# Yuki-11/CSBSR

Hardware: AMD Instinct MI355X
Metric: training imgs/s (448->1792 x4, PSPNet) (higher is better)
Workload: dtype fp16 storage / fp32 accumulate (detector forward: split fp16 hi+lo); 1 GPU; CSBSR KBPN x4 + PSPNet, beta=0.3, joint phase (iter 40000), per-GPU batch 8, LR 448x448 -> HR 1792x1792, fwd+loss+bwd+Adam; batch resident in HBM (H2D outside `value`, timed beside it as with_h2d_inside_step); full-size synthetic crack images degraded on the device; global_batch=8, micro_batch=8, parallelism=dp1

## Files before the change

### csbsr_amd/_lib.py

```python
import ctypes as C
import os
from collections import namedtuple

import torch

_HERE = os.path.dirname(os.path.abspath(__file__))
LIB_PATH = os.environ.get("CSBSR_LIB") or os.path.join(_HERE, "libcsbsr_hip.so")

ACT_NONE, ACT_RELU, ACT_LRELU, ACT_PRELU, ACT_SIGMOID = 0, 1, 2, 3, 4
RES_NONE, RES_ADD, RES_SUB, RES_MUL, RES_FMA = 0, 1, 2, 3, 4
STAT_NONE, STAT_BN, STAT_SAMPLE_SUM = 0, 1, 2

i32, i64, f32, vp = C.c_int32, C.c_int64, C.c_float, C.c_void_p


class Seg(C.Structure):
    _fields_ = [("ptr", vp), ("sn", i64), ("sy", i64), ("sx", i64), ("c", i32), ("creal", i32)]


class ConvDesc(C.Structure):
    _fields_ = [("inp", Seg * 2), ("N", i32), ("H", i32), ("W", i32), ("OH", i32), ("OW", i32),
                ("transposed", i32), ("KH", i32), ("KW", i32), ("stride", i32), ("pad", i32), ("dil", i32),
                ("wt", vp), ("cout", i32), ("coutp", i32),
                ("out16", vp), ("o_sn", i64), ("o_sy", i64), ("o_sx", i64),
# ... 31 lines not shown
    _fields_ = [("npix", i64), ("hw", i64), ("c", i32), ("creal", i32),
                ("x", vp), ("x_ld", i64), ("mean", vp), ("invstd", vp), ("gamma", vp), ("beta", vp),
                ("res", vp), ("res_ld", i64), ("act", i32), ("_pad", i32), ("prelu", vp), ("drop", vp),
                ("y", vp), ("y_ld", i64), ("dy", vp), ("dy_ld", i64), ("red", vp), ("dprelu", vp),
                ("dx", vp), ("dx_ld", i64), ("dres", vp), ("dres_ld", i64), ("dres_accumulate", i32), ("_pad1", i32),
                ("dgamma", vp), ("dbeta", vp), ("x_lo", i64), ("res_lo", i64), ("y_lo", i64)]


SIGNATURES = {
    "csbsr_version": (i32, []),
    "csbsr_last_error": (C.c_char_p, []),
    "csbsr_conv_forward": (i32, [C.POINTER(ConvDesc), vp]),
    "csbsr_conv_wgrad": (i32, [C.POINTER(WgradDesc), vp]),
    "csbsr_conv_hr_eligible": (i32, [C.POINTER(ConvDesc)]),
    "csbsr_conv_hr_forward": (i32, [C.POINTER(ConvDesc), vp]),
    "csbsr_conv_x3_eligible": (i32, [C.POINTER(ConvDesc)]),
    "csbsr_conv_x3_forward": (i32, [C.POINTER(ConvDesc), vp]),
    "csbsr_packed_weight_elems_x3": (i64, [i32, i32]),
    "csbsr_pack_weights_x3": (i32, [vp, vp, i32, i32, i32, i32, i32, i32, i32, vp]),
    "csbsr_conv_x3n_eligible": (i32, [C.POINTER(ConvDesc)]),
    "csbsr_conv_x3n_forward": (i32, [C.POINTER(ConvDesc), vp]),
    "csbsr_packed_weight_elems_x3n": (i64, [i32, i32]),
    "csbsr_pack_weights_x3n": (i32, [vp, vp, i32, i32, i32, i32, i32, i32, i32, i32, i32, C.c_float, vp]),
    "csbsr_conv_x3w_eligible": (i32, [C.POINTER(ConvDesc)]),
    "csbsr_conv_x3w_forward": (i32, [C.POINTER(ConvDesc), vp]),
    "csbsr_packed_weight_elems_x3w": (i64, [i32, i32]),
    "csbsr_pack_weights_x3w": (i32, [vp, vp, i32, i32, i32, i32, i32, i32, i32, vp]),
    "csbsr_packed_weight_elems_x3_strided": (i64, [i32, i32, i32]),
    "csbsr_pack_weights_x3_strided": (i32, [vp, vp, i32, i32, i32, i32, i32, i32, i32, i32, vp]),
    "csbsr_conv_tp_eligible": (i32, [C.POINTER(ConvDesc)]),
    "csbsr_conv_tp_forward": (i32, [C.POINTER(ConvDesc), vp]),
    "csbsr_packed_weight_elems_tp": (i64, [i32, i32]),
    "csbsr_pack_weights_tp": (i32, [vp, vp, i32, i32, i32, i32, i32, i32, i32, i32, i32, i32, vp]),
    "csbsr_packed_weight_elems_hr": (i64, [i32, i32, i32]),
    "csbsr_pack_weights_hr": (i32, [vp, vp, i32, i32, i32, i32, i32, i32, i32, i32, vp]),
    "csbsr_packed_weight_elems": (i64, [i32] * 9),
    "csbsr_pack_weights": (i32, [vp, vp] + [i32] * 12 + [vp]),
    "csbsr_packed_weight_elems_split": (i64, [i32] * 9),
    "csbsr_pack_weights_split": (i32, [vp, vp] + [i32] * 11 + [f32, i32, vp]),
    "csbsr_axpby_split": (i32, [i64, i32, vp, i64, i64, f32, vp, i64, i64, f32, vp, i64, i64, vp]),
    "csbsr_nchw32_to_nhwc16_split": (i32, [vp, vp, i32, i32, i32, i32, i32, i64, i64, vp, vp, vp]),
    "csbsr_maxpool3x3s2_fwd_split": (i32, [vp, i64, i64, vp, i64, i64, i32, i32, i32, i32, vp]),
    "csbsr_maxpool3x3s2_bwd_split": (i32, [vp, i64, i64, vp, i64, i64, vp, vp, i32, i32, i32, i32, vp]),
    "csbsr_adaptive_avgpool_fwd_split": (i32, [vp, i64, i64, vp, i64, i64, i32, i32, i32, i32, i32, i32, vp]),
    "csbsr_sum_act_split": (i32, [i64, i32, i32, vp, vp, vp, vp, i64, i64, i32, vp]),
    "csbsr_weighted_pool_fwd_split": (i32, [vp, i64, i64, vp, vp, i32, i64, i32, vp]),
    "csbsr_bilinear_fwd_split": (i32, [vp, i64, i64, vp, i64, i64, i32, i32, i32, i32, i32, i32, i32, vp, vp]),
    "csbsr_unpack_wgrad": (i32, [vp, vp] + [i32] * 9 + [f32, i32, i32, vp]),
    "csbsr_wgrad_splits": (i32, [i32, i32, i64]),
    "csbsr_wgrad_splits_desc": (i32, [vp]),
    "csbsr_epilogue_backward": (i32, [C.POINTER(EpiBwdDesc), vp]),
    "csbsr_set_reduction_scratch": (i32, [vp, i64]),
    "csbsr_axpby": (i32, [i64, i32, vp, i64, f32, vp, i64, f32, vp, i64, vp]),
    "csbsr_fill_f16": (i32, [vp, i64, i32, i64, f32, vp]),
    "csbsr_sum_act": (i32, [i64, i32, i32, vp, vp, vp, i64, i32, vp]),
    "csbsr_weighted_pool_fwd": (i32, [vp, i64, vp, vp, i32, i64, i32, vp]),
    "csbsr_weighted_pool_bwd": (i32, [vp, i64, vp, vp, vp, i64, vp, i32, i64, i32, vp]),
    "csbsr_nchw32_to_nhwc16": (i32, [vp, vp, i32, i32, i32, i32, i32, i64, vp, vp, vp]),
    "csbsr_nhwc16_to_nchw32": (i32, [vp, i64, vp, i32, i32, i32, i32, f32, f32, vp]),
    "csbsr_plane_reduce": (i32, [vp, vp, i32, i64, vp, vp]),
    "csbsr_channel_mean_sub": (i32, [vp, i64, i64, i64, i32, i32, i32, i32, i32, vp, vp]),
    "csbsr_thin_tp_backward_slabs": (i32, [i32, i32]),
    "csbsr_conv_thin_dact_eligible": (i32, [vp]),
    "csbsr_conv_split_fused_eligible": (i32, [C.POINTER(ConvDesc)]),
    "csbsr_thin_tp_backward": (i32, [vp, i64, i64, i64, vp, i64, i64, i64, vp, i32, i32, i32, i32, vp, i32, i32, i32, vp, i64, i64, i64, vp, vp, vp]),
    "csbsr_conv_pair1x1_slabs": (i32, [i32, i32, i32, vp]),
    "csbsr_conv_pair1x1_backward": (i32, [vp, i64, i64, i64, vp, i64, i64, i64, vp, f32, i32, i32, i32, vp, i64, i64, i64, vp, vp]),
    "csbsr_round_weights": (i32, [vp, vp, vp, i32, i32, i32, i32, i32, vp]),
    "csbsr_dc_bias": (i32, [vp, i32, i32, vp, i64, i32, vp, i64, i32, vp, i32, vp, vp]),
    "csbsr_instnorm_bwd": (i32, [vp, i64, vp, vp, vp, vp, i32, i32, i32, i64, vp, vp]),
    "csbsr_border_class_fill": (i32, [vp, vp, i64, i32, i32, i32, i32, vp]),
    "csbsr_border_class_fill_masked": (i32, [vp, vp, i64, vp, i64, C.c_float, i32, i32, i32, i32, vp]),
    "csbsr_border_class_sums": (i32, [vp, i64, vp, i32, i32, i32, i32, vp]),
    "csbsr_border_class_fill_masked_sums": (i32, [vp, vp, i64, vp, i64, C.c_float, vp, i32, i32, i32, i32, vp]),
    "csbsr_border_class_sums_prelu": (i32, [vp, i64, vp, i64, vp, vp, i32, i32, i32, i32, vp]),
    "csbsr_ring_class_sums": (i32, [vp, i64, vp, i32, i32, i32, i32, vp]),
    "csbsr_bn_finalize": (i32, [vp, i64, i32, i32, f32, f32, vp, vp, vp, vp, vp]),
    "csbsr_bn_apply": (i32, [C.POINTER(BnDesc), vp]),
    "csbsr_bn_backward": (i32, [C.POINTER(BnDesc), vp]),
    "csbsr_maxpool3x3s2_fwd": (i32, [vp, vp, i32, i32, i32, i32, vp]),
    "csbsr_maxpool3x3s2_bwd": (i32, [vp, vp, vp, vp, i32, i32, i32, i32, vp]),
    "csbsr_adaptive_avgpool_fwd": (i32, [vp, i64, vp, i32, i32, i32, i32, i32, i32, vp]),
    "csbsr_adaptive_avgpool_bwd": (i32, [vp, vp, i64, i32, i32, i32, i32, i32, i32, i32, vp]),
    "csbsr_bilinear_fwd": (i32, [vp, i64, vp, i64, i32, i32, i32, i32, i32, i32, i32, vp, vp]),
    "csbsr_bilinear_bwd": (i32, [vp, i64, vp, i64, i32, i32, i32, i32, i32, i32, i32, i32, vp, vp]),
    "csbsr_bilinear32_fwd": (i32, [vp, vp, i32, i32, i32, i32, i32, i32, vp]),
    "csbsr_bilinear32_bwd": (i32, [vp, vp, i32, i32, i32, i32, i32, i32, vp]),
    "csbsr_bicubic_up_add": (i32, [vp, vp, i32, i32, i32, i32, vp]),
    "csbsr_aa_bicubic_up": (i32, [vp, vp, i32, i32, i32, i32, i32, i32, vp]),
    "csbsr_aa_bicubic_down_fwd": (i32, [vp, vp, i32, i32, i32, i32, i32, vp]),
    "csbsr_aa_bicubic_down_bwd": (i32, [vp, vp, i32, i32, i32, i32, i32, i32, vp]),
    "csbsr_area_down_fwd": (i32, [vp, vp, i32, i32, i32, i32, vp]),
    "csbsr_area_down_bwd": (i32, [vp, vp, i32, i32, i32, i32, i32, vp]),
    "csbsr_blur_fwd": (i32, [vp, vp, i32, i32, i32, i32, i32, i32, vp, vp, vp, i64, vp]),
    "csbsr_blur_bwd_input": (i32, [vp, vp, vp, i32, i32, i32, i32, i32, i32, i32, vp]),
    "csbsr_blur_bwd_kernel": (i32, [vp, vp, vp, i32, i32, i32, i32, i32, i32, vp]),
    "csbsr_sdf": (i32, [vp, vp, vp, i32, i32, i32, vp]),
    "csbsr_crack_weight": (i32, [vp, vp, vp, vp, i32, i32, i32, f32, f32, i32, vp]),
    "csbsr_segloss_reduce": (i32, [vp, vp, vp, i32, i64, vp, f32, f32, vp]),
    "csbsr_segloss_finish": (i32, [vp, vp, vp, i32, i64, vp, f32, f32, f32, f32, f32, f32, vp, vp, vp, i32, vp]),
    "csbsr_l1_fwd_bwd": (i32, [vp, vp, vp, i32, i32, i64, vp, f32, vp, vp, i32, vp]),
    "csbsr_sigmoid_bwd_to_nhwc8": (i32, [vp, vp, vp, i64, f32, vp]),
    "csbsr_gaussian_kernels": (i32, [vp, vp, i32, i32, vp]),
    "csbsr_gather_crop_u8": (i32, [vp, vp, vp, i32, vp, i32, i32, i32, vp, vp]),
    "csbsr_gather_resize_u8": (i32, [vp, vp, vp, i32, vp, i32, i32, i32, i32, vp, vp]),
    "csbsr_stitch_clip_u8": (i32,[vp, i32, i32, i32, i32, i32, i32, i32, vp, vp, vp]),
    "csbsr_stitch_tiles_u8": (i32, [vp, i32, i32, i32, i32, vp, vp, vp, i32, vp, vp, vp]),
    "csbsr_threshold_planes_u8": (i32, [vp, vp, i32, i64, i32, vp, vp]),
    "csbsr_iou_sweep": (i32, [vp, vp, vp, i32, i64, i32, f32, vp, vp, vp, vp, vp]),
    "csbsr_psnr_ssim": (i32, [vp, vp, i32, i32, i32, i32, vp, vp, vp, vp]),
    "csbsr_surface_prepare": (i32, [vp, vp, vp, i32, i32, i32, vp, vp, vp, vp, vp, vp, vp]),
    "csbsr_surface_gather": (i32, [vp, vp, vp, vp, i32, i32, i32, i32, vp, vp, vp, vp, vp, i32, vp, i32, vp, vp]),
    "csbsr_pr_sweep": (i32, [vp, vp, vp, i32, i32, i32, i32, i32, vp, vp, vp]),
    "csbsr_skeleton_max_passes": (i32, []),
    "csbsr_skeleton_init": (i32, [vp, f32, i32, i32, i32, vp, vp]),
    "csbsr_skeleton_passes": (i32, [vp, vp, i32, i32, i32, i32, vp, vp]),
    "csbsr_skeleton_finish": (i32, [vp, i32, i32, i32, vp, vp]),
    "csbsr_centerline_counts": (i32, [vp, vp, f32, vp, vp, i32, i32, i32, vp, vp]),
    "csbsr_ccl_tile": (i32, [C.POINTER(i32), C.POINTER(i32)]),
    "csbsr_ccl_label": (i32, [vp, f32, i32, i32, i32, i32, vp, vp, vp]),
    "csbsr_component_sums": (i32, [vp, vp, i32, i32, i32, vp, vp]),
    "csbsr_component_keep": (i32, [vp, vp, i32, i32, i32, i32, vp, vp, vp]),
    "csbsr_width_max_radius": (i32, []),
    "csbsr_width_tile": (i32, [C.POINTER(i32), C.POINTER(i32)]),
    "csbsr_skeleton_width": (i32, [vp, f32, vp, i32, i32, i32, i32, vp, vp, vp]),
    "csbsr_component_width": (i32, [vp, vp, i32, i32, i32, vp, vp]),
    "csbsr_skeleton_topology": (i32, [vp, i32, i32, i32, vp, vp, vp]),
    "csbsr_component_topology": (i32, [vp, vp, vp, i32, i32, i32, vp, vp]),
    "csbsr_branch_tile": (i32, [C.POINTER(i32), C.POINTER(i32)]),
    "csbsr_branch_label": (i32, [vp, i32, i32, i32, vp, vp, vp]),
    "csbsr_branch_sums": (i32, [vp, vp, vp, vp, i32, i32, i32, vp, vp]),
    "csbsr_prune_max_spur": (i32, []),
    "csbsr_prune_steps": (i32, [C.POINTER(i32), C.POINTER(i32)]),
    "csbsr_prune_tile": (i32, [C.POINTER(i32), C.POINTER(i32)]),
    "csbsr_prune_work_bytes": (i64, [i32, i32, i32]),
    "csbsr_skeleton_prune": (i32, [vp, i32, i32, i32, i32, vp, vp, vp, vp, vp]),
    "csbsr_head1_fwd":(i32, [vp, i64, i64, i32, vp, vp, i32, vp, i64, vp]),
    "csbsr_head1_bwd_input": (i32, [vp, i64, vp, i32, vp, i64, i64, vp]),
    "csbsr_adam_step": (i32, [vp, vp, vp, i32, C.c_double, C.c_double, C.c_float, vp]),
    "csbsr_sgd_step": (i32, [vp, vp, vp, i32, C.c_double, C.c_double, C.c_double, vp]),
    "csbsr_fingerprint": (i32, [vp, vp, vp, i32, vp, vp]),
}

DEBUG_SIGNATURES = {
    "csbsr_debug_set_wgrad_tr": (None, [i32]),
    "csbsr_debug_set_conv_glds": (None, [i32]),
    "csbsr_debug_set_conv_tp": (None, [i32]),
    "csbsr_debug_set_conv_x3": (None, [i32]),
    "csbsr_debug_set_conv_x3w": (None, [i32]),
    "csbsr_debug_set_conv_x3n": (None, [i32]),
    "csbsr_debug_set_wgrad_hr": (None, [i32]),
    "csbsr_debug_last_conv_kernel": (i32, []),
    "csbsr_debug_last_wgrad_kernel": (i32, []),
    "csbsr_debug_cu_trace": (i32, [vp, i32, i32, vp]),
    "csbsr_debug_stream_create_cu_mask": (i32, [C.POINTER(vp), C.POINTER(C.c_uint32), i32]),
    "csbsr_debug_stream_destroy": (i32, [vp]),
    "csbsr_debug_stream_set_cu_budget": (i32, [vp, i32]),
    "csbsr_debug_stream_cu_budget": (i32, [vp]),
}

Hook = namedtuple("Hook", "var default attr parse setter setter_parse", defaults=(None, None, None, None, int))
_not0, _is1 = "0".__ne__, "1".__eq__
ENV_HOOKS = (
    Hook("CSBSR_WGRAD_DBG", setter="csbsr_debug_set_wgrad_tr"),
    Hook("CSBSR_CONV_X3", "1", "use_x3", _not0, "csbsr_debug_set_conv_x3"),
    Hook("CSBSR_CONV_X3W", "0", "use_x3w", lambda v: {"0": 0, "all": 2}.get(v, 1), "csbsr_debug_set_conv_x3w", lambda v: 1 if v == "all" else int(v)),
# ... 52 lines not shown
```

### csbsr_amd/modeling/pspnet.py

```python
import os

import torch

from .. import _lib as L
from ..engine import FM, Conv, _ptr
from .blocks import ConvBN, act_bwd, sft_bwd
from .kbpn import border_tap_mask
from .shapes import RESNET34

DROP_P = {"drop_1": 0.3, "drop_2a": 0.15, "drop_2b": 0.15, "drop_2c": 0.15, "aux_drop": 0.1}
DROP_C = {"drop_1": 1024, "drop_2a": 256, "drop_2b": 64, "drop_2c": 64, "aux_drop": 256}


class _SFTLike:

    def __init__(self, eng, P, pre, cf, cconst):
        def mk(name, act, prelu):
            return Conv(eng, f"{pre}.{name}.layer", P, 3, 1, 1, bias=True, act=act, prelu=f"{pre}.{name}.act.weight" if prelu else False,
                        split=(cf, cconst) if prelu else None)
        self.sc0, self.sc1 = mk("conv_scale.0", L.ACT_PRELU, True), mk("conv_scale.1", L.ACT_SIGMOID, False)
        self.sh0, self.sh1 = mk("conv_shift.0", L.ACT_PRELU, True), mk("conv_shift.1", L.ACT_NONE, False)

    def convs(self):
        return [self.sc0, self.sc1, self.sh0, self.sh1]


class _ResBlock:

    def __init__(self, eng, P, pre, stride, dil, down, layer):
        self.eng, self.layer = eng, layer
        self.c1 = ConvBN(eng, P, pre + ".conv1", pre + ".bn1", 3, stride, dil, dil)
        self.c2 = ConvBN(eng, P, pre + ".conv2", pre + ".bn2", 3, 1, dil, dil)
        self.down = ConvBN(eng, P, pre + ".downsample.0", pre + ".downsample.1", 1, stride, 0, act=L.ACT_NONE) if down else None

    def units(self):
        return [self.c1, self.c2] + ([self.down] if self.down else [])

    def fwd(self, x, training, tape, out=None):
        a1 = self.c1.fwd(x, training, tape)
        pre = self.c2.conv_stats(a1, training)
        res = self.down.fwd(x, training, tape) if self.down else x
        return self.c2.fwd(a1, training, tape, res=res, out=out, pre=pre)

    def bwd(self, tape, dy):
        dres = self.eng.new(dy.N, dy.H, dy.W, dy.c)
        da1 = self.c2.bwd(tape, dy, dres=dres)
        g1 = self.c1.bwd_bn(tape, da1)
        del da1
        dx = self.down.bwd(tape, dres) if self.down else dres
        self.c1.bwd_dx(g1, out=dx, acc=True)
        return dx


class PSPNet:
    drop_keys = tuple(DROP_P)

    def __init__(self, eng, params, prefix="segmentation_model", blur_dim=None):
        self.eng, self.P, self.prefix = eng, params, prefix
        self.blur_dim = blur_dim
        self.blur_skip = []
        e, P, f = eng, params, prefix + ".feats"
        if blur_dim is not None:
            for i in range(2):
                bs = f"{prefix}.blur_skip.{2 * i + 1}"
                self.blur_skip.append((_SFTLike(e, P, f"{prefix}.blur_skip.{2 * i}", 64, blur_dim), ConvBN(e, P, bs + ".layer", bs + ".norm", 3)))
            self.Mtap = border_tap_mask().to(eng.device)
        self.stem = ConvBN(e, P, f + ".conv1", f + ".bn1", 7, 2)
        self.blocks = []
        inpl = 64
        for li, (planes, nblk, stride, dil) in enumerate(RESNET34, 1):
            for b in range(nblk):
                s_, d_ = (stride, 1) if b == 0 else (1, dil)
                self.blocks.append(_ResBlock(e, P, f"{f}.layer{li}.{b}", s_, d_, b == 0 and (stride != 1 or inpl != planes), li))
            inpl = planes
        self.x3_block = [b for b in self.blocks if b.layer == 3][-1]
        self.psp_convs = [Conv(e, f"{prefix}.psp.stages.{i}.1", P, 1, bias=False) for i in range(4)]
        self.bottleneck = Conv(e, prefix + ".psp.bottleneck", P, 1, bias=True, act=L.ACT_RELU)
        self.ups = [ConvBN(e, P, f"{prefix}.{n}.conv.0", f"{prefix}.{n}.conv.1", 3, bias=True, act=L.ACT_PRELU, prelu=P[f"{prefix}.{n}.conv.2.weight"])
                    for n in ("up_1", "up_2", "up_3")]
        self.final = Conv(e, prefix + ".final.0", P, 1, bias=True, act=L.ACT_SIGMOID)
        self.aux0 = ConvBN(e, P, prefix + ".aux.0", prefix + ".aux.1", 3)
        self.aux4 = Conv(e, prefix + ".aux.4", P, 1, bias=True, act=L.ACT_SIGMOID)
        self.saved = None
        self.split = False
        self.split_tail_plain = int(os.environ.get("CSBSR_SPLIT_TAIL_PLAIN", "0"))

    def all_convs(self):
        cs = [u.conv for u in [self.stem] + [u for b in self.blocks for u in b.units()]]
        cs += self.psp_convs + [self.bottleneck] + [u.conv for u in self.ups] + [self.final, self.aux0.conv, self.aux4]
        for sft, cb in self.blur_skip:
            cs += sft.convs() + [cb.conv]
        return cs

    def invalidate(self):
        for c in self.all_convs():
            c.invalidate()

    def make_dropout(self, B, training, enabled=True):
        if not training or not enabled:
            return {k: None for k in DROP_P}
        out = {}
        for k, p in DROP_P.items():
            keep = (torch.rand(B, DROP_C[k], device=self.eng.device) >= p).to(torch.float32) / (1.0 - p)
            out[k] = keep.contiguous()
        return out

    def forward(self, xin, drop, training=True, kvec=None):
        e = self.eng
        B, H, W = xin.N, xin.H, xin.W
        tape = {} if training and torch.is_grad_enabled() else None
        trunk = tape if self.blur_dim is None else None
        a = self.stem.fwd(xin, training, trunk)
        PH, PW = (a.H + 2 - 3) // 2 + 1, (a.W + 2 - 3) // 2 + 1
        x = e.new(B, PH, PW, 64, split=bool(a.lo))
        L.call("csbsr_maxpool3x3s2_fwd_split", _ptr(a.t), a.ld, a.lo, _ptr(x.t), x.ld, x.lo, B, a.H, a.W, 64, e.stream)
        pool = (a, x)
        for blk in self.blocks:
            out = None
            if blk is self.blocks[-1]:
                cat = e.new(B, x.H, x.W, 2560, split=bool(x.lo))
                out = cat.slice(2048, 2560)
            x = blk.fwd(x, training, trunk, out=out)
            if blk is self.x3_block:
                x3 = x
        fH, fW = x.H, x.W
        psp = []
        for i, size in enumerate((1, 2, 3, 6)):
            pooled = e.new(B, size, size, 512, split=bool(x.lo))
            L.call("csbsr_adaptive_avgpool_fwd_split", _ptr(x.t), x.ld, x.lo, _ptr(pooled.t), pooled.ld, pooled.lo, B, fH, fW, 512, size, size,
                   e.stream)
            pc = self.psp_convs[i].fwd(pooled)
            e.bilinear(pc, fH, fW, False, out=cat.slice(512 * i, 512 * (i + 1)))
            psp.append((pooled, pc))
        bott = self.bottleneck.fwd(cat)
        cur, cur_drop = bott, drop["drop_1"]
        ups = []
        for j, (up, name) in enumerate(zip(self.ups, ("drop_2a", "drop_2b", "drop_2c"))):
            if cur.lo and j >= len(self.ups) - self.split_tail_plain:
                cur = FM(cur.t, cur.c, H=cur.H, W=cur.W)
            u = e.bilinear(cur, cur.H * 2, cur.W * 2, False, drop=cur_drop)
            ups.append((cur, cur_drop))
            cur, cur_drop = up.fwd(u, training, trunk, drop=drop[name] if j == 2 else None), drop[name]
        if trunk is not None:
            tape.update(pool=pool, psp=(cat, psp, bott), ups=ups)
        if self.blur_dim is not None:
            cur = self._blur_skip_fwd(cur, kvec, training, tape)
        seg32 = e.f32(B, 1, H, W, zero=False)
        self.final.fwd(cur, out32=seg32)
        aa = self.aux0.fwd(x3, training, trunk, drop=drop["aux_drop"])
        aux_lo = e.f32(B, 1, x3.H, x3.W, zero=False)
        self.aux4.fwd(aa, out32=aux_lo)
        aux32 = e.f32(B, 1, H, W, zero=False)
        L.call("csbsr_bilinear32_fwd", _ptr(aux_lo), _ptr(aux32), B, x3.H, x3.W, H, W, 1, e.stream)
        if tape is not None:
            tape.update(seg32=seg32, p3=cur)
        if trunk is not None:
            tape["aux"] = (aa, aux_lo)
        self.saved = tape
        return seg32, aux32

    def _blur_skip_fwd(self, p, kvec, training, tape):
        e = self.eng
        q, bsv = p, []
        for sft, cb in self.blur_skip:
            t1, f1 = sft.sc0.fwd_folded(q, kvec, self.Mtap)
            sc = sft.sc1.fwd(t1)
            t2, f2 = sft.sh0.fwd_folded(q, kvec, self.Mtap)
            y = sft.sh1.fwd(t2, res=q, res2=sc, res_mode=L.RES_FMA)
            bsv.append((q, (t1, f1, sc, t2, f2, y)))
            q = cb.fwd(y, training, tape)
        out = e.new(p.N, p.H, p.W, p.c, split=bool(p.lo))
        L.call("csbsr_axpby_split", p.npix, p.cp, _ptr(p.t), p.ld, p.lo, 1.0, _ptr(q.t), q.ld, q.lo, 1.0, _ptr(out.t), out.ld, out.lo,
               e.stream)
        if tape is not None:
            tape["blur_skip"] = bsv
        return out

    def _blur_skip_bwd(self, tape, d):
        bsv = tape.pop("blur_skip")
        for i in (1, 0):
            sft, cb = self.blur_skip[i]
            q, saves = bsv.pop()
            dy = cb.bwd(tape, d)
            del d
            dq = self.eng.new(q.N, q.H, q.W, q.c) if i > 0 else None
            sft_bwd(sft.sc0, sft.sc1, sft.sh0, sft.sh1, saves, q, dy, self.Mtap, dx=dq)
            del dy, saves
            d = dq

    def _sigmoid_head_bwd(self, conv, dprob32, prob32, x, frozen=False):
        e = self.eng
        B, _, H, W = prob32.shape
        dpre = e.new(B, H, W, 1)
        L.call("csbsr_sigmoid_bwd_to_nhwc8", _ptr(dprob32), _ptr(prob32), _ptr(dpre.t), B * H * W, 1.0, e.stream)
        if not frozen:
            act_bwd(conv, dpre)
            conv.bwd_weights(dpre, x)
        return conv.bwd_input(dpre)

    def backward(self, dseg32, daux32, need_dxin=True):
        e = self.eng
        tape, self.saved = self.saved, None
        B, _, H, W = dseg32.shape
        if self.blur_dim is not None:
            self._blur_skip_bwd(tape, self._sigmoid_head_bwd(self.final, dseg32, tape.pop("seg32"), tape.pop("p3"), frozen=True))
            return None
        aa, aux_lo = tape.pop("aux")
        daux_lo = e.f32(B, 1, *aux_lo.shape[2:], zero=False)
        L.call("csbsr_bilinear32_bwd", _ptr(daux32), _ptr(daux_lo), B, *aux_lo.shape[2:], H, W, 1, e.stream)
        dx3_aux = self.aux0.bwd(tape, self._sigmoid_head_bwd(self.aux4, daux_lo, aux_lo, aa))
        del aa
        d = self._sigmoid_head_bwd(self.final, dseg32, tape.pop("seg32"), tape.pop("p3"))
        ups = tape.pop("ups")
        for up in reversed(self.ups):
            cur, cur_drop = ups.pop()
            du = up.bwd(tape, d)
            d = e.new(B, cur.H, cur.W, cur.c)
            e.bilinear_bwd(du, d, False, False, drop=cur_drop)
            del du, cur
        cat, psp, bott = tape.pop("psp")
        act_bwd(self.bottleneck, d, bott)
        self.bottleneck.bwd_weights(d, cat)
        dcat = self.bottleneck.bwd_input(d)
        del d, bott
        fH, fW = cat.H, cat.W
        dy = dcat.slice(2048, 2560)
        for i, size in enumerate((1, 2, 3, 6)):
            pooled, pc = psp[i]
            dpc = e.new(B, size, size, 512)
            e.bilinear_bwd(dcat.slice(512 * i, 512 * (i + 1)), dpc, False, False)
            self.psp_convs[i].bwd_weights(dpc, pooled)
            dpool = self.psp_convs[i].bwd_input(dpc)
            L.call("csbsr_adaptive_avgpool_bwd", _ptr(dpool.t), _ptr(dy.t), dy.ld, 1, B, fH, fW, 512, size, size, e.stream)
        del cat, psp
        for blk in reversed(self.blocks):
            if blk is self.x3_block:
                L.call("csbsr_axpby", dy.npix, dy.cp, _ptr(dy.t), dy.ld, 1.0, _ptr(dx3_aux.t), dx3_aux.ld, 1.0, _ptr(dy.t), dy.ld, e.stream)
            dy = blk.bwd(tape, dy)
        a, p = tape.pop("pool")
        da = e.new(B, a.H, a.W, 64)
        assert dy.flat_ok() and dy.ld == dy.cp
        L.call("csbsr_maxpool3x3s2_bwd_split", _ptr(a.t), a.ld, a.lo, _ptr(p.t), p.ld, p.lo, _ptr(dy.t), _ptr(da.t), B, a.H, a.W, 64, e.stream)
        return self.stem.bwd(tape, da, need_dx=need_dxin)
```

### include/csbsr_hip.h

```cpp
#ifndef CSBSR_HIP_H
#define CSBSR_HIP_H
#include <stdint.h>
#ifdef __cplusplus
extern "C" {
#endif

typedef void* csbsr_stream_t;

int csbsr_version(void);
const char* csbsr_last_error(void);

enum { CSBSR_ACT_NONE = 0, CSBSR_ACT_RELU = 1, CSBSR_ACT_LRELU = 2, CSBSR_ACT_PRELU = 3, CSBSR_ACT_SIGMOID = 4 };
enum { CSBSR_RES_NONE = 0, CSBSR_RES_ADD = 1, CSBSR_RES_SUB = 2, CSBSR_RES_MUL = 3, CSBSR_RES_FMA = 4 };
enum { CSBSR_STAT_NONE = 0, CSBSR_STAT_BN = 1 ,
       CSBSR_STAT_SAMPLE_SUM = 2  };

typedef struct {
  const void* ptr;
  int64_t sn, sy, sx;
  int32_t c;
  int32_t creal;
} csbsr_seg_t;

typedef struct {
// ... 148 lines not shown

int csbsr_axpby_split(int64_t npix, int32_t c, const void* x, int64_t x_ld, int64_t x_lo, float a, const void* z, int64_t z_ld,
                      int64_t z_lo, float b, void* y, int64_t y_ld, int64_t y_lo, csbsr_stream_t s);
int csbsr_nchw32_to_nhwc16_split(const float* src, void* dst, int32_t N, int32_t C, int32_t H, int32_t W, int32_t cp,
                                 int64_t dst_ld, int64_t dst_lo, const float* mean, const float* invstd, csbsr_stream_t s);
int csbsr_maxpool3x3s2_fwd_split(const void* x, int64_t x_ld, int64_t x_lo, void* y, int64_t y_ld, int64_t y_lo, int32_t N,
                                 int32_t H, int32_t W, int32_t c, csbsr_stream_t s);
int csbsr_maxpool3x3s2_bwd_split(const void* x, int64_t x_ld, int64_t x_lo, const void* y, int64_t y_ld, int64_t y_lo,
                                 const void* dy, void* dx, int32_t N, int32_t H, int32_t W, int32_t c, csbsr_stream_t s);
int csbsr_adaptive_avgpool_fwd_split(const void* x, int64_t x_ld, int64_t x_lo, void* y, int64_t y_ld, int64_t y_lo, int32_t N,
                                     int32_t H, int32_t W, int32_t c, int32_t OH, int32_t OW, csbsr_stream_t s);
int csbsr_sum_act_split(int64_t npix, int32_t c, int32_t n, const void* const* xs, const int64_t* x_lds, const int64_t* x_los, void* y,
                        int64_t y_ld, int64_t y_lo, int32_t relu, csbsr_stream_t s);
int csbsr_weighted_pool_fwd_split(const void* x, int64_t x_ld, int64_t x_lo, const float* w, float* out, int32_t N, int64_t hw,
                                  int32_t c, csbsr_stream_t s);
int csbsr_bilinear_fwd_split(const void* x, int64_t x_ld, int64_t x_lo, void* y, int64_t y_ld, int64_t y_lo, int32_t N, int32_t H,
                             int32_t W, int32_t c, int32_t OH, int32_t OW, int32_t align_corners, const float* drop,
                             csbsr_stream_t s);

int csbsr_sum_act(int64_t npix, int32_t c, int32_t n, const void* const* xs, const int64_t* x_lds, void* y, int64_t y_ld,
                  int32_t relu, csbsr_stream_t s);
int csbsr_weighted_pool_fwd(const void* x, int64_t x_ld, const float* w, float* out, int32_t N, int64_t hw, int32_t c,
                            csbsr_stream_t s);
int csbsr_weighted_pool_bwd(const void* x, int64_t x_ld, const float* w, const float* dout, void* dx, int64_t dx_ld, float* dw,
                            int32_t N, int64_t hw, int32_t c, csbsr_stream_t s);

int csbsr_nchw32_to_nhwc16(const float* src, void* dst, int32_t N, int32_t C, int32_t H, int32_t W, int32_t cp,
                           int64_t dst_ld, const float* mean, const float* invstd, csbsr_stream_t s);
int csbsr_nhwc16_to_nchw32(const void* src, int64_t src_ld, float* dst, int32_t N, int32_t C, int32_t H, int32_t W,
                           float alpha, float beta, csbsr_stream_t s);
int csbsr_plane_reduce(const float* a, const float* b, int32_t planes, int64_t hw, float* out, csbsr_stream_t s);
int csbsr_channel_mean_sub(const void* x, int64_t sn, int64_t sy, int64_t sx, int32_t N, int32_t H, int32_t W, int32_t cp,
                           int32_t step, float* out, csbsr_stream_t s);
int csbsr_round_weights(const float* w, float* wq, float* S, int32_t D0, int32_t D1, int32_t KH, int32_t KW, int32_t mode, csbsr_stream_t s);
int csbsr_dc_bias(const float* S, int32_t cout, int32_t cin, const float* m0, int64_t m0_ld, int32_t c0, const float* m1, int64_t m1_ld,
                  int32_t c1, const float* bias, int32_t N, float* out, csbsr_stream_t s);
int csbsr_instnorm_bwd(const void* dy, int64_t dy_ld, const float* x, const float* mean, const float* invstd,
                       float* dx, int32_t accumulate, int32_t N, int32_t C, int64_t hw, float* red,
                       csbsr_stream_t s);

int csbsr_border_class_fill(const float* V, void* out, int64_t ld, int32_t N, int32_t H, int32_t W, int32_t c,
                            csbsr_stream_t s);
int csbsr_border_class_fill_masked(const float* V, void* out, int64_t ld, const void* mask, int64_t mask_ld, float mask_slope, int32_t N,
                                   int32_t H, int32_t W, int32_t c, csbsr_stream_t s);
int csbsr_border_class_sums(const void* x, int64_t ld, float* sums, int32_t N, int32_t H, int32_t W, int32_t c,
                            csbsr_stream_t s);
int csbsr_border_class_fill_masked_sums(const float* V, void* out, int64_t ld, const void* mask, int64_t mask_ld, float mask_slope,
                                        float* sums, int32_t N, int32_t H, int32_t W, int32_t c, csbsr_stream_t s);
int csbsr_border_class_sums_prelu(const void* x, int64_t ld, const void* t, int64_t t_ld, float* sums, float* negdot, int32_t N, int32_t H,
                                  int32_t W, int32_t c, csbsr_stream_t s);
int csbsr_ring_class_sums(const void* x, int64_t ld, float* sums, int32_t N, int32_t H, int32_t W, int32_t c,
                          csbsr_stream_t s);

int csbsr_bn_finalize(const float* stat, int64_t count, int32_t c, int32_t cstride, float eps, float momentum,
                      float* mean, float* invstd, float* running_mean, float* running_var, csbsr_stream_t s);
typedef struct {
  int64_t npix, hw;
  int32_t c, creal;
  const void* x; int64_t x_ld;
  const float *mean, *invstd, *gamma, *beta;
  const void* res; int64_t res_ld;
  int32_t act; int32_t _pad;
  const float* prelu;
  const float* drop;
  void* y; int64_t y_ld;
  const void* dy; int64_t dy_ld;
  float* red;
  float* dprelu;
  void* dx; int64_t dx_ld;
  void* dres; int64_t dres_ld; int32_t dres_accumulate; int32_t _pad1;
  float *dgamma, *dbeta;
  int64_t x_lo, res_lo, y_lo;
} csbsr_bn_desc_t;
int csbsr_bn_apply(const csbsr_bn_desc_t* d, csbsr_stream_t s);
int csbsr_bn_backward(const csbsr_bn_desc_t* d, csbsr_stream_t s);

int csbsr_maxpool3x3s2_fwd(const void* x, void* y, int32_t N, int32_t H, int32_t W, int32_t c, csbsr_stream_t s);
int csbsr_maxpool3x3s2_bwd(const void* x, const void* y, const void* dy, void* dx, int32_t N, int32_t H, int32_t W,
                           int32_t c, csbsr_stream_t s);
int csbsr_adaptive_avgpool_fwd(const void* x, int64_t x_ld, void* y, int32_t N, int32_t H, int32_t W, int32_t c,
                               int32_t OH, int32_t OW, csbsr_stream_t s);
int csbsr_adaptive_avgpool_bwd(const void* dy, void* dx, int64_t dx_ld, int32_t accumulate, int32_t N, int32_t H,
                               int32_t W, int32_t c, int32_t OH, int32_t OW, csbsr_stream_t s);
int csbsr_bilinear_fwd(const void* x, int64_t x_ld, void* y, int64_t y_ld, int32_t N, int32_t H, int32_t W,
                       int32_t c, int32_t OH, int32_t OW, int32_t align_corners, const float* drop, csbsr_stream_t s);
int csbsr_bilinear_bwd(const void* dy, int64_t dy_ld, void* dx, int64_t dx_ld, int32_t accumulate, int32_t N,
                       int32_t H, int32_t W, int32_t c, int32_t OH, int32_t OW, int32_t align_corners,
                       const float* drop, csbsr_stream_t s);
int csbsr_bilinear32_fwd(const float* x, float* y, int32_t planes, int32_t H, int32_t W, int32_t OH, int32_t OW,
                         int32_t align_corners, csbsr_stream_t s);
int csbsr_bilinear32_bwd(const float* dy, float* dx, int32_t planes, int32_t H, int32_t W, int32_t OH, int32_t OW,
                         int32_t align_corners, csbsr_stream_t s);
int csbsr_bicubic_up_add(const float* x, float* out, int32_t planes, int32_t H, int32_t W, int32_t scale,
                         csbsr_stream_t s);
int csbsr_aa_bicubic_up(const float* x, float* y, int32_t planes, int32_t H, int32_t W, int32_t scale,
                        int32_t antialias, int32_t clip, csbsr_stream_t s);
int csbsr_aa_bicubic_down_fwd(const float* x, float* y, int32_t planes, int32_t H, int32_t W, int32_t f,
                              int32_t antialias, csbsr_stream_t s);
int csbsr_aa_bicubic_down_bwd(const float* dy, float* dx, int32_t accumulate, int32_t planes, int32_t H, int32_t W,
                              int32_t f, int32_t antialias, csbsr_stream_t s);
int csbsr_area_down_fwd(const float* x, float* y, int32_t planes, int32_t H, int32_t W, int32_t f, csbsr_stream_t s);
int csbsr_area_down_bwd(const float* dy, float* dx, int32_t accumulate, int32_t planes, int32_t H, int32_t W, int32_t f,
                        csbsr_stream_t s);

int csbsr_blur_fwd(const float* x, const float* kvec, int32_t N, int32_t C, int32_t H, int32_t W, int32_t K,
                   int32_t stride, const float* sub, float* y32, void* y16, int64_t y16_ld, csbsr_stream_t s);
int csbsr_blur_bwd_input(const float* dy, const float* kvec, float* dx, int32_t accumulate, int32_t N, int32_t C,
                         int32_t H, int32_t W, int32_t K, int32_t stride, csbsr_stream_t s);
int csbsr_blur_bwd_kernel(const float* dy, const float* x, float* dk, int32_t N, int32_t C, int32_t H, int32_t W,
                          int32_t K, int32_t stride, csbsr_stream_t s);

int csbsr_sdf(const float* mask, float* sdf, float* scratch, int32_t N, int32_t H, int32_t W, csbsr_stream_t s);
int csbsr_crack_weight(const float* mask, float* w_hr, float* w_lr, float* scratch, int32_t N, int32_t H, int32_t W,
                       float amp, float lambda, int32_t scale, csbsr_stream_t s);
int csbsr_segloss_reduce(const float* p, const float* t, const float* sdf, int32_t N, int64_t hw, float* sums,
                         float pw0, float pw1, csbsr_stream_t s);
int csbsr_segloss_finish(const float* p, const float* t, const float* sdf, int32_t N, int64_t hw, const float* sums,
                         float alpha, float pw0, float pw1, float lw0, float lw1, float weight, const float* gscale,
                         float* loss, float* dp, int32_t dp_accumulate, csbsr_stream_t s);
int csbsr_l1_fwd_bwd(const float* a, const float* b, const float* wmap, int32_t N, int32_t C, int64_t hw,
                     float* sums, float gscale, const float* gs_n, float* da, int32_t da_accumulate, csbsr_stream_t s);
int csbsr_sigmoid_bwd_to_nhwc8(const float* dp, const float* p, void* out, int64_t npix, float scale,
                               csbsr_stream_t s);

int csbsr_head1_fwd(const void* x, int64_t ld, int64_t lo, int32_t c, const float* w, const float* bias, int32_t sigmoid, float* out,
                    int64_t npix, csbsr_stream_t s);
int csbsr_head1_bwd_input(const void* dpre, int64_t dpre_ld, const float* w, int32_t c, void* dx, int64_t ld, int64_t npix, csbsr_stream_t s);

int csbsr_gaussian_kernels(const float* params, float* out, int32_t N, int32_t K, csbsr_stream_t s);
int csbsr_gather_crop_u8(const uint8_t* pool, const int64_t* offsets, const int32_t* dims, int32_t channels, const int32_t* sel,
                         int32_t B, int32_t h, int32_t w, float* out, csbsr_stream_t s);
int csbsr_gather_resize_u8(const uint8_t* pool, const int64_t* offsets, const int32_t* dims, int32_t channels, const int32_t* sel,
                           int32_t B, int32_t h, int32_t w, int32_t antialias, float* out, csbsr_stream_t s);
int csbsr_stitch_clip_u8(const float* patches, int32_t B, int32_t C, int32_t nH, int32_t nW, int32_t ph, int32_t pw, int32_t clip,
                         float* out_f32, uint8_t* out_u8, csbsr_stream_t s);
int csbsr_stitch_tiles_u8(const float* patches, int32_t N, int32_t C, int32_t PH, int32_t PW, const int32_t* tiles, const int64_t* offsets,
                          const int32_t* dims, int32_t clip, float* out_f32, uint8_t* out_u8, csbsr_stream_t s);
int csbsr_threshold_planes_u8(const float* pred, const float* thresholds, int32_t N, int64_t hw, int32_t S, uint8_t* out, csbsr_stream_t s);
int csbsr_iou_sweep(const float* pred, const float* mask, const float* thresholds, int32_t N, int64_t hw, int32_t T, float smooth,
                    uint32_t* hist, float* iou, float* inter, float* uni, csbsr_stream_t s);
int csbsr_psnr_ssim(const float* a, const float* b, int32_t N, int32_t C, int32_t H, int32_t W, float* sums, float* psnr, float* ssim,
                    csbsr_stream_t s);

int csbsr_surface_prepare(const float* pred, const float* mask, const float* thresholds, int32_t H, int32_t W, int32_t T, uint8_t* lvl,
                          uint8_t* gt, int32_t* counts, int32_t* rowflag, uint16_t* gcol, int32_t* dgt, csbsr_stream_t s);
int csbsr_surface_gather(const uint8_t* lvl, const uint8_t* gt, const int32_t* dgt, const int32_t* rowflag, int32_t H, int32_t W, int32_t j0,
                         int32_t nj, uint16_t* gcol, const int32_t* tab_off, const int32_t* tab_cap, int32_t* tab_keys, uint32_t* tab_cnt,
                         int32_t max_cap, int32_t* rows, int32_t max_rows, int32_t* meta, csbsr_stream_t s);

int csbsr_pr_sweep(const float* pred, const float* mask, const float* thresholds, int32_t N, int32_t H, int32_t W, int32_t T, int32_t tol2,
                   uint32_t* hist, int32_t* counts, csbsr_stream_t s);

int32_t csbsr_skeleton_max_passes(void);
int csbsr_skeleton_init(const float* planes, float threshold, int32_t N, int32_t H, int32_t W, uint32_t* work, csbsr_stream_t s);
int csbsr_skeleton_passes(const uint32_t* src, uint32_t* dst, int32_t N, int32_t H, int32_t W, int32_t passes, int32_t* deleted,
                          csbsr_stream_t s);
int csbsr_skeleton_finish(const uint32_t* work, int32_t N, int32_t H, int32_t W, uint8_t* out, csbsr_stream_t s);
int csbsr_centerline_counts(const uint8_t* skel_pred, const float* pred, float threshold, const uint8_t* skel_gt, const float* mask, int32_t N,
                            int32_t H, int32_t W, int32_t* counts, csbsr_stream_t s);

int csbsr_ccl_tile(int32_t* th, int32_t* tw);
int csbsr_ccl_label(const float* planes, float threshold, int32_t N, int32_t H, int32_t W, int32_t connectivity, int32_t* work,
                    int32_t* labels, csbsr_stream_t s);
int csbsr_component_sums(const int32_t* labels, const uint8_t* skeleton, int32_t N, int32_t H, int32_t W, int32_t* acc, csbsr_stream_t s);
int csbsr_component_keep(const int32_t* labels, const int32_t* acc, int32_t N, int32_t H, int32_t W, int32_t min_px, uint8_t* keep,
                         int32_t* labels_out, csbsr_stream_t s);
// ... 39 lines not shown
```

Measured before the change: 8.296 imgs/s.

## Fuse PSP pyramid pooling and bilinear backward across all four levels

```diff
diff --git a/csbsr_amd/_lib.py b/csbsr_amd/_lib.py
--- a/csbsr_amd/_lib.py
+++ b/csbsr_amd/_lib.py
@@ -137,6 +137,9 @@
     "csbsr_maxpool3x3s2_bwd": (i32, [vp, vp, vp, vp, i32, i32, i32, i32, vp]),
     "csbsr_adaptive_avgpool_fwd": (i32, [vp, i64, vp, i32, i32, i32, i32, i32, i32, vp]),
     "csbsr_adaptive_avgpool_bwd": (i32, [vp, vp, i64, i32, i32, i32, i32, i32, i32, i32, vp]),
+    "csbsr_psp_pool_fwd": (i32, [vp, i64, i64, vp, vp, vp, i32, i32, i32, i32, vp]),
+    "csbsr_psp_pool_bwd": (i32, [vp, vp, i64, i32, i32, i32, i32, i32, vp]),
+    "csbsr_psp_bilinear_bwd": (i32, [vp, i64, vp, vp, i32, i32, i32, i32, vp]),
     "csbsr_bilinear_fwd": (i32, [vp, i64, vp, i64, i32, i32, i32, i32, i32, i32, i32, vp, vp]),
     "csbsr_bilinear_bwd": (i32, [vp, i64, vp, i64, i32, i32, i32, i32, i32, i32, i32, i32, vp, vp]),
     "csbsr_bilinear32_fwd": (i32, [vp, vp, i32, i32, i32, i32, i32, i32, vp]),
diff --git a/csbsr_amd/csrc/psp_passes.hip b/csbsr_amd/csrc/psp_passes.hip
--- /dev/null
+++ b/csbsr_amd/csrc/psp_passes.hip
@@ -0,0 +1,261 @@
+#include "common.h"
+
+#define ST(s) reinterpret_cast<hipStream_t>(s)
+#define PSP_LEVELS 4
+#define PSP_BINS 50
+#define PSP_BATCH 8
+
+static __host__ __device__ __forceinline__ int prior(int l) { return l == 3 ? 6 : l + 1; }
+static __device__ __forceinline__ int bin_first(int l) { return l == 0 ? 0 : l == 1 ? 1 : l == 2 ? 5 : 14; }
+static __device__ __forceinline__ int level_of_bin(int b) { return b < 1 ? 0 : b < 5 ? 1 : b < 14 ? 2 : 3; }
+static __device__ __forceinline__ int bin_lo(int o, int n, int S) { return (o * n) / S; }
+static __device__ __forceinline__ int bin_hi(int o, int n, int S) { return ((o + 1) * n + S - 1) / S; }
+
+static __device__ __forceinline__ void st_split(half_t* p, long lo, const float (&v)[8]) {
+  h8 a, b;
+#pragma unroll
+  for (int e = 0; e < 8; ++e) { a[e] = (half_t)v[e]; b[e] = (half_t)(v[e] - (float)a[e]); }
+  *reinterpret_cast<h8*>(p) = a;
+  if (lo) *reinterpret_cast<h8*>(p + lo) = b;
+}
+static __device__ __forceinline__ void bil_src(int o, int in, int out, int& i0, int& i1, float& w1) {
+  float src = (o + 0.5f) * ((float)in / (float)out) - 0.5f;
+  if (src < 0.f) src = 0.f;
+  i0 = (int)src; if (i0 > in - 1) i0 = in - 1;
+  i1 = i0 + 1 < in ? i0 + 1 : in - 1;
+  w1 = src - i0;
+}
+
+struct PspMaps { half_t* p[PSP_LEVELS]; long ld[PSP_LEVELS]; long lo[PSP_LEVELS]; };
+struct PspGrads { const half_t* p[PSP_LEVELS]; };
+struct PspSlices { const half_t* p[PSP_LEVELS]; int scan[PSP_LEVELS]; };
+
+static __device__ __forceinline__ void psp_block(int N, int groups, int& n, int& g, int& l, int& o0, int& o1) {
+  int b = blockIdx.x;
+  g = b % groups; b /= groups;
+  n = b % N; b /= N;
+  l = level_of_bin(b);
+  o0 = (b - bin_first(l)) / prior(l); o1 = (b - bin_first(l)) % prior(l);
+}
+static __device__ __forceinline__ float lane_sum(const float (*sred)[8][8], int cl, int e) {
+  float s_ = 0.f;
+  for (int q = 0; q < 32; ++q) s_ += sred[q][cl][e];
+  return s_;
+}
+
+__global__ __launch_bounds__(256) void psp_pool_fwd_kernel(const half_t* x, long x_ld, long x_lo, const PspMaps out, int N, int H, int W, int c8) {
+  __shared__ float sred[32][8][8];
+  int n, g, l, oy, ox;
+  psp_block(N, (c8 + 7) / 8, n, g, l, oy, ox);
+  const int S = prior(l);
+  const int cl = threadIdx.x & 7, pl = threadIdx.x >> 3;
+  const int cc = g * 8 + cl;
+  const int y0 = bin_lo(oy, H, S), y1 = bin_hi(oy, H, S);
+  const int x0 = bin_lo(ox, W, S), x1 = bin_hi(ox, W, S);
+  const int bw = x1 - x0, cnt = (y1 - y0) * bw;
+  const bool block = (long)(H / S) * (W / S) >= 64;
+  const int step = block ? 32 : 1, first = block ? pl : (pl == 0 ? 0 : cnt);
+  float a[8];
+#pragma unroll
+  for (int e = 0; e < 8; ++e) a[e] = 0.f;
+  if (cc < c8) {
+    const half_t* base = x + (long)n * H * W * x_ld + cc * 8;
+    for (int i0 = first; i0 < cnt; i0 += step * PSP_BATCH) {
+      h8 vh[PSP_BATCH], vl[PSP_BATCH];
+#pragma unroll
+      for (int u = 0; u < PSP_BATCH; ++u) {
+        const int i = i0 + u * step;
+        if (i < cnt) {
+          const half_t* p = base + ((long)(y0 + i / bw) * W + (x0 + i % bw)) * x_ld;
+          vh[u] = *reinterpret_cast<const h8*>(p);
+          if (x_lo) vl[u] = *reinterpret_cast<const h8*>(p + x_lo);
+        }
+      }
+#pragma unroll
+      for (int u = 0; u < PSP_BATCH; ++u)
+        if (i0 + u * step < cnt) {
+          float v[8];
+#pragma unroll
+          for (int e = 0; e < 8; ++e) v[e] = (float)vh[u][e];
+          if (x_lo) {
+#pragma unroll
+            for (int e = 0; e < 8; ++e) v[e] += (float)vl[u][e];
+          }
+#pragma unroll
+          for (int e = 0; e < 8; ++e) a[e] += v[e];
+        }
+    }
+  }
+#pragma unroll
+  for (int e = 0; e < 8; ++e) sred[pl][cl][e] = a[e];
+  __syncthreads();
+  if (pl == 0 && cc < c8) {
+    half_t* q = out.p[l] + (((long)n * S + oy) * S + ox) * out.ld[l] + cc * 8;
+    if (block) {
+      float o[8];
+#pragma unroll
+      for (int e = 0; e < 8; ++e) o[e] = lane_sum(sred, cl, e) / cnt;
+      st_split(q, out.lo[l], o);
+    } else {
+      const float inv = 1.f / ((y1 - y0) * (x1 - x0));
+#pragma unroll
+      for (int e = 0; e < 8; ++e) a[e] *= inv;
+      st_split(q, out.lo[l], a);
+    }
+  }
+}
+
+__global__ __launch_bounds__(256) void psp_pool_bwd_kernel(const PspGrads dpool, half_t* dx, long dx_ld, int accumulate, int H, int W, int c8) {
+  const int n = (int)blockIdx.y / H, iy = (int)blockIdx.y % H;
+  const unsigned i = blockIdx.x * 256u + threadIdx.x;
+  if (i >= (unsigned)W * (unsigned)c8) return;
+  const int ix = (int)(i / (unsigned)c8), cc = (int)(i - (unsigned)ix * (unsigned)c8);
+  half_t* q = dx + (((long)n * H + iy) * W + ix) * dx_ld + cc * 8;
+  h8 cur = {0, 0, 0, 0, 0, 0, 0, 0};
+  if (accumulate) cur = *reinterpret_cast<const h8*>(q);
+#pragma unroll
+  for (int l = 0; l < PSP_LEVELS; ++l) {
+    const int S = prior(l);
+    const half_t* dy = dpool.p[l];
+    float a[8];
+#pragma unroll
+    for (int e = 0; e < 8; ++e) a[e] = 0.f;
+    for (int oy = 0; oy < S; ++oy) {
+      const int y0 = bin_lo(oy, H, S), y1 = bin_hi(oy, H, S);
+      if (iy < y0 || iy >= y1) continue;
+      for (int ox = 0; ox < S; ++ox) {
+        const int x0 = bin_lo(ox, W, S), x1 = bin_hi(ox, W, S);
+        if (ix < x0 || ix >= x1) continue;
+        const h8 gv = *reinterpret_cast<const h8*>(dy + ((((long)n * S + oy) * S + ox) * c8 + cc) * 8);
+        const float inv = 1.f / ((y1 - y0) * (x1 - x0));
+#pragma unroll
+        for (int e = 0; e < 8; ++e) a[e] += (float)gv[e] * inv;
+      }
+    }
+    if (l > 0 || accumulate) {
+#pragma unroll
+      for (int e = 0; e < 8; ++e) a[e] += (float)cur[e];
+    }
+#pragma unroll
+    for (int e = 0; e < 8; ++e) cur[e] = (half_t)a[e];
+  }
+  *reinterpret_cast<h8*>(q) = cur;
+}
+
+__global__ __launch_bounds__(256) void psp_bilinear_bwd_kernel(const PspSlices dys, long dy_ld, const PspMaps dxs, int N, int OH, int OW, int c8) {
+  __shared__ float sred[32][8][8];
+  int n, g, l, iy, ix;
+  psp_block(N, (c8 + 7) / 8, n, g, l, iy, ix);
+  if (dys.scan[l] < 0) return;
+  const int H = prior(l), W = H;
+  const half_t* dy = dys.p[l];
+  const int cl = threadIdx.x & 7, pl = threadIdx.x >> 3;
+  const int cc = g * 8 + cl;
+  const float ry = (float)OH / H, rx = (float)OW / W;
+  int oy_lo = (int)floorf((iy - 1.5f) * ry) - 2, oy_hi = (int)ceilf((iy + 1.5f) * ry) + 2;
+  int ox_lo = (int)floorf((ix - 1.5f) * rx) - 2, ox_hi = (int)ceilf((ix + 1.5f) * rx) + 2;
+  if (iy == 0) oy_lo = 0;
+  if (ix == 0) ox_lo = 0;
+  if (iy == H - 1) oy_hi = OH - 1;
+  if (ix == W - 1) ox_hi = OW - 1;
+  oy_lo = oy_lo < 0 ? 0 : oy_lo; ox_lo = ox_lo < 0 ? 0 : ox_lo;
+  oy_hi = oy_hi > OH - 1 ? OH - 1 : oy_hi; ox_hi = ox_hi > OW - 1 ? OW - 1 : ox_hi;
+  const int ww = ox_hi - ox_lo + 1, cnt = (oy_hi - oy_lo + 1) * ww;
+  const int step = dys.scan[l] ? 1 : 32, first = dys.scan[l] ? (pl == 0 ? 0 : cnt) : pl;
+  float a[8];
+#pragma unroll
+  for (int e = 0; e < 8; ++e) a[e] = 0.f;
+  if (cc < c8) {
+    const half_t* base = dy + (long)n * OH * OW * dy_ld + cc * 8;
+    for (int i0 = first; i0 < cnt; i0 += step * PSP_BATCH) {
+      h8 gv[PSP_BATCH];
+      float wv[PSP_BATCH];
+#pragma unroll
+      for (int u = 0; u < PSP_BATCH; ++u) {
+        const int i = i0 + u * step;
+        wv[u] = 0.f;
+        if (i < cnt) {
+          const int oy = oy_lo + i / ww, ox = ox_lo + i % ww;
+          int y0, y1, x0, x1; float wy, wx;
+          bil_src(oy, H, OH, y0, y1, wy); bil_src(ox, W, OW, x0, x1, wx);
+          float cy = 0.f, cx = 0.f;
+          if (y0 == iy) cy += 1.f - wy;
+          if (y1 == iy) cy += wy;
+          if (x0 == ix) cx += 1.f - wx;
+          if (x1 == ix) cx += wx;
+          wv[u] = cy * cx;
+          if (wv[u] != 0.f) gv[u] = *reinterpret_cast<const h8*>(base + ((long)oy * OW + ox) * dy_ld);
+        }
+      }
+#pragma unroll
+      for (int u = 0; u < PSP_BATCH; ++u)
+        if (wv[u] != 0.f) {
+          const float w_ = wv[u];
+#pragma unroll
+          for (int e = 0; e < 8; ++e) a[e] += w_ * (float)gv[u][e];
+        }
+    }
+  }
+#pragma unroll
+  for (int e = 0; e < 8; ++e) sred[pl][cl][e] = a[e];
+  __syncthreads();
+  if (pl == 0 && cc < c8) {
+    h8 o;
+#pragma unroll
+    for (int e = 0; e < 8; ++e) o[e] = (half_t)(lane_sum(sred, cl, e) + 0.f);
+    *reinterpret_cast<h8*>(dxs.p[l] + (((long)n * H + iy) * W + ix) * dxs.ld[l] + cc * 8) = o;
+  }
+}
+
+extern "C" int csbsr_psp_pool_fwd(const void* x, int64_t x_ld, int64_t x_lo, void* const* ys, const int64_t* y_lds, const int64_t* y_los,
+                                  int32_t N, int32_t H, int32_t W, int32_t c, csbsr_stream_t s) {
+  CSBSR_CHECK(x && ys && y_lds && y_los && c > 0 && c % 8 == 0 && N > 0 && H > 0 && W > 0, "psp_pool_fwd: bad args");
+  PspMaps out;
+  for (int l = 0; l < PSP_LEVELS; ++l) {
+    CSBSR_CHECK(ys[l], "psp_pool_fwd: bad args");
+    out.p[l] = (half_t*)ys[l]; out.ld[l] = y_lds[l]; out.lo[l] = y_los[l];
+  }
+  const int c8 = c / 8, groups = (c8 + 7) / 8;
+  CSBSR_CHECK((long)N * PSP_BINS * groups < (1l << 31), "psp_pool_fwd: size");
+  hipLaunchKernelGGL(psp_pool_fwd_kernel, dim3(N * PSP_BINS * groups), dim3(256), 0, ST(s), (const half_t*)x, x_ld, x_lo, out, N, H, W, c8);
+  CSBSR_LAUNCH_CHECK("csbsr_psp_pool_fwd");
+  return 0;
+}
+
+extern "C" int csbsr_psp_pool_bwd(const void* const* dpools, void* dx, int64_t dx_ld, int32_t accumulate, int32_t N, int32_t H, int32_t W,
+                                  int32_t c, csbsr_stream_t s) {
+  CSBSR_CHECK(dpools && dx && c > 0 && c % 8 == 0 && N > 0 && H > 0 && W > 0 && (long)N * H <= 65535 && (long)W * (c / 8) < (1l << 31),
+              "psp_pool_bwd: bad args");
+  PspGrads g;
+  for (int l = 0; l < PSP_LEVELS; ++l) { CSBSR_CHECK(dpools[l], "psp_pool_bwd: bad args"); g.p[l] = (const half_t*)dpools[l]; }
+  const long per_row = (long)W * (c / 8);
+  hipLaunchKernelGGL(psp_pool_bwd_kernel, dim3((unsigned)((per_row + 255) / 256), (unsigned)(N * H)), dim3(256), 0, ST(s), g, (half_t*)dx, dx_ld,
+                     accumulate, H, W, c / 8);
+  CSBSR_LAUNCH_CHECK("csbsr_psp_pool_bwd");
+  return 0;
+}
+
+extern "C" int csbsr_psp_bilinear_bwd(const void* const* dys, int64_t dy_ld, void* const* dxs, const int64_t* dx_lds, int32_t N, int32_t OH,
+                                      int32_t OW, int32_t c, csbsr_stream_t s) {
+  CSBSR_CHECK(dys && dxs && dx_lds && c > 0 && c % 8 == 0 && N > 0 && OH > 0 && OW > 0, "psp_bilinear_bwd: bad args");
+  PspSlices in;
+  PspMaps out;
+  const int c8 = c / 8, groups = (c8 + 7) / 8;
+  int fused = 0;
+  for (int l = 0; l < PSP_LEVELS; ++l) {
+    CSBSR_CHECK(dys[l] && dxs[l], "psp_bilinear_bwd: bad args");
+    const int S = prior(l);
+    in.p[l] = (const half_t*)dys[l]; out.p[l] = (half_t*)dxs[l]; out.ld[l] = dx_lds[l]; out.lo[l] = 0;
+    const long strips = (long)N * ((S + 7) / 8), per_row = (long)S * c8;
+    if ((long)(OH / S) * (OW / S) >= 64) in.scan[l] = 0;
+    else if (OH >= S && OW >= S && 2 * OH <= 5 * S && 2 * OW <= 5 * S && strips <= 65535 && (per_row + 255) / 256 * strips >= 64) in.scan[l] = -1;
+    else in.scan[l] = 1;
+    if (in.scan[l] < 0) { if (int e = csbsr_bilinear_bwd(dys[l], dy_ld, dxs[l], dx_lds[l], 0, N, S, S, c, OH, OW, 0, nullptr, s)) return e; }
+    else ++fused;
+  }
+  if (!fused) return 0;
+  CSBSR_CHECK((long)N * PSP_BINS * groups < (1l << 31), "psp_bilinear_bwd: size");
+  hipLaunchKernelGGL(psp_bilinear_bwd_kernel, dim3(N * PSP_BINS * groups), dim3(256), 0, ST(s), in, dy_ld, out, N, OH, OW, c8);
+  CSBSR_LAUNCH_CHECK("csbsr_psp_bilinear_bwd");
+  return 0;
+}
diff --git a/csbsr_amd/modeling/psp_passes.py b/csbsr_amd/modeling/psp_passes.py
--- /dev/null
+++ b/csbsr_amd/modeling/psp_passes.py
@@ -0,0 +1,36 @@
+import ctypes as C
+
+from .. import _lib as L
+from ..engine import _ptr
+
+PRIORS = (1, 2, 3, 6)
+
+
+def _ptrs(ts):
+    return (C.c_void_p * 4)(*[t.data_ptr() for t in ts])
+
+
+def _i64s(vs):
+    return (C.c_int64 * 4)(*[int(v) for v in vs])
+
+
+def pool_fwd(eng, x, channels=512):
+    pooled = [eng.new(x.N, s, s, channels, split=bool(x.lo)) for s in PRIORS]
+    L.call("csbsr_psp_pool_fwd", _ptr(x.t), x.ld, x.lo, _ptrs([p.t for p in pooled]), _i64s([p.ld for p in pooled]),
+           _i64s([p.lo for p in pooled]), x.N, x.H, x.W, channels, eng.stream)
+    return pooled
+
+
+def bilinear_bwd(eng, dcat, channels=512):
+    dys = [dcat.slice(channels * i, channels * (i + 1)) for i in range(4)]
+    dpcs = [eng.new(dcat.N, s, s, channels) for s in PRIORS]
+    assert all(d.flat_ok() for d in dys)
+    L.call("csbsr_psp_bilinear_bwd", _ptrs([d.t for d in dys]), dcat.ld, _ptrs([d.t for d in dpcs]), _i64s([d.ld for d in dpcs]),
+           dcat.N, dcat.H, dcat.W, channels, eng.stream)
+    return dpcs
+
+
+def pool_bwd(eng, dpools, dy, channels=512):
+    for d, s in zip(dpools, PRIORS):
+        assert d.ld == channels and d.flat_ok() and (d.H, d.W) == (s, s)
+    L.call("csbsr_psp_pool_bwd", _ptrs([d.t for d in dpools]), _ptr(dy.t), dy.ld, 1, dy.N, dy.H, dy.W, channels, eng.stream)
diff --git a/csbsr_amd/modeling/pspnet.py b/csbsr_amd/modeling/pspnet.py
--- a/csbsr_amd/modeling/pspnet.py
+++ b/csbsr_amd/modeling/pspnet.py
@@ -4,6 +4,7 @@
 
 from .. import _lib as L
 from ..engine import FM, Conv, _ptr
+from . import psp_passes
 from .blocks import ConvBN, act_bwd, sft_bwd
 from .kbpn import border_tap_mask
 from .shapes import RESNET34
@@ -84,6 +85,7 @@
         self.saved = None
         self.split = False
         self.split_tail_plain = int(os.environ.get("CSBSR_SPLIT_TAIL_PLAIN", "0"))
+        self.psp_one_pass = True
 
     def all_convs(self):
         cs = [u.conv for u in [self.stem] + [u for b in self.blocks for u in b.units()]]
@@ -125,10 +127,14 @@
                 x3 = x
         fH, fW = x.H, x.W
         psp = []
+        pools = psp_passes.pool_fwd(e, x) if self.psp_one_pass else None
         for i, size in enumerate((1, 2, 3, 6)):
-            pooled = e.new(B, size, size, 512, split=bool(x.lo))
-            L.call("csbsr_adaptive_avgpool_fwd_split", _ptr(x.t), x.ld, x.lo, _ptr(pooled.t), pooled.ld, pooled.lo, B, fH, fW, 512, size, size,
-                   e.stream)
+            if pools is not None:
+                pooled = pools[i]
+            else:
+                pooled = e.new(B, size, size, 512, split=bool(x.lo))
+                L.call("csbsr_adaptive_avgpool_fwd_split", _ptr(x.t), x.ld, x.lo, _ptr(pooled.t), pooled.ld, pooled.lo, B, fH, fW, 512, size, size,
+                       e.stream)
             pc = self.psp_convs[i].fwd(pooled)
             e.bilinear(pc, fH, fW, False, out=cat.slice(512 * i, 512 * (i + 1)))
             psp.append((pooled, pc))
@@ -225,13 +231,24 @@
         del d, bott
         fH, fW = cat.H, cat.W
         dy = dcat.slice(2048, 2560)
+        dpcs = psp_passes.bilinear_bwd(e, dcat) if self.psp_one_pass else None
+        dpools = []
         for i, size in enumerate((1, 2, 3, 6)):
             pooled, pc = psp[i]
-            dpc = e.new(B, size, size, 512)
-            e.bilinear_bwd(dcat.slice(512 * i, 512 * (i + 1)), dpc, False, False)
+            if dpcs is not None:
+                dpc = dpcs[i]
+            else:
+                dpc = e.new(B, size, size, 512)
+                e.bilinear_bwd(dcat.slice(512 * i, 512 * (i + 1)), dpc, False, False)
             self.psp_convs[i].bwd_weights(dpc, pooled)
             dpool = self.psp_convs[i].bwd_input(dpc)
-            L.call("csbsr_adaptive_avgpool_bwd", _ptr(dpool.t), _ptr(dy.t), dy.ld, 1, B, fH, fW, 512, size, size, e.stream)
+            if dpcs is not None:
+                dpools.append(dpool)
+            else:
+                L.call("csbsr_adaptive_avgpool_bwd", _ptr(dpool.t), _ptr(dy.t), dy.ld, 1, B, fH, fW, 512, size, size, e.stream)
+        if dpcs is not None:
+            psp_passes.pool_bwd(e, dpools, dy)
+        del dpcs, dpools
         del cat, psp
         for blk in reversed(self.blocks):
             if blk is self.x3_block:
diff --git a/include/csbsr_hip.h b/include/csbsr_hip.h
--- a/include/csbsr_hip.h
+++ b/include/csbsr_hip.h
@@ -254,6 +254,12 @@
                                int32_t OH, int32_t OW, csbsr_stream_t s);
 int csbsr_adaptive_avgpool_bwd(const void* dy, void* dx, int64_t dx_ld, int32_t accumulate, int32_t N, int32_t H,
                                int32_t W, int32_t c, int32_t OH, int32_t OW, csbsr_stream_t s);
+int csbsr_psp_pool_fwd(const void* x, int64_t x_ld, int64_t x_lo, void* const* ys, const int64_t* y_lds, const int64_t* y_los,
+                       int32_t N, int32_t H, int32_t W, int32_t c, csbsr_stream_t s);
+int csbsr_psp_pool_bwd(const void* const* dpools, void* dx, int64_t dx_ld, int32_t accumulate, int32_t N, int32_t H, int32_t W,
+                       int32_t c, csbsr_stream_t s);
+int csbsr_psp_bilinear_bwd(const void* const* dys, int64_t dy_ld, void* const* dxs, const int64_t* dx_lds, int32_t N, int32_t OH,
+                           int32_t OW, int32_t c, csbsr_stream_t s);
 int csbsr_bilinear_fwd(const void* x, int64_t x_ld, void* y, int64_t y_ld, int32_t N, int32_t H, int32_t W,
                        int32_t c, int32_t OH, int32_t OW, int32_t align_corners, const float* drop, csbsr_stream_t s);
 int csbsr_bilinear_bwd(const void* dy, int64_t dy_ld, void* dx, int64_t dx_ld, int32_t accumulate, int32_t N,
```

Measured after the change: 8.340 imgs/s (median of 6 runs). Within noise of the previous version (+0.5%).
